# ToKe79/nuts333

Measured on NVIDIA B200. Metric: rendered messages/sec (colour+swear+ban), higher is better.
Workload: dtype u8

## Files before the change

nuts333_b200/csrc/nutsb_kernels.cuh:

```cuda
#pragma once
#include "nutsb_common.cuh"


struct OpsView {
    i64 n;
    const u8  *text;
    const u64 *toff;
    const u8  *kind;
    const i32 *target;
    const i32 *except_user;
    const u8  *flags;
    const i32 *gate;
    const u8  *verdict;
};

struct PopView {
    i32 n_users, n_rooms, n_rooms_tot;
    const i32 *user_room;
    const i32 *user_cls;
    const i32 *user_slot;
    const i32 *slot_user;
    const u8  *slot_cf;
    const u8  *slot_lv;
    const i32 *room_slot_off;
// ... 864 lines not shown
#endif
#ifndef NUTSB_FAN_GROUP
#define NUTSB_FAN_GROUP 1
#endif
#define NUTSB_FAN_SMEM (NUTSB_FAN_ON_CAP + 80 + NUTSB_FAN_OFF_CAP + 80 + 16 * NUTSB_FAN_RUN_CAP)

struct FanoutArgs {
    const ItemDesc *items; const uint4 *runs;
    const u8 *slab; u64 off_base;
    u8 *out;
};

__device__ __forceinline__ void nutsb_fanout_block(const FanoutArgs &A, u32 item, u8 *s_dyn)
{
    u8 *const s_on = s_dyn;
    u8 *const s_off = s_dyn + NUTSB_FAN_ON_CAP + 80;
    uint4 *const s_run = (uint4 *)(s_dyn + NUTSB_FAN_ON_CAP + 80 + NUTSB_FAN_OFF_CAP + 80);
    const int tid = threadIdx.x, warp = tid >> 5;
    const ItemDesc d = A.items[item];
    const bool staged = d.on_len <= NUTSB_FAN_ON_CAP && d.off_len <= NUTSB_FAN_OFF_CAP;
    const u32 a_on = (u32)(d.on_src & 15), a_off = (u32)(d.off_src & 15);
    if (staged) {
        const uint4 *g = (const uint4 *)(A.slab + (d.on_src - a_on));
        for (u32 v = (u32)tid, nv = (a_on + d.on_len + 15) >> 4; v < nv; v += NUTSB_FAN_THREADS) ((uint4 *)s_on)[v] = __ldg(g + v);
        g = (const uint4 *)(A.slab + (d.off_src - a_off));
        for (u32 v = (u32)tid, nv = (a_off + d.off_len + 15) >> 4; v < nv; v += NUTSB_FAN_THREADS) ((uint4 *)s_off)[v] = __ldg(g + v);
    }
    for (u32 r0 = 0; r0 < d.run_cnt; r0 += NUTSB_FAN_RUN_CAP) {
        const u32 nr = d.run_cnt - r0 < NUTSB_FAN_RUN_CAP ? d.run_cnt - r0 : NUTSB_FAN_RUN_CAP;
        if (r0) __syncthreads();
        for (u32 r = (u32)tid; r < nr; r += NUTSB_FAN_THREADS) s_run[r] = __ldg(A.runs + d.run_begin + r0 + r);
        __syncthreads();
        for (u32 r = (u32)warp / NUTSB_FAN_GROUP; r < nr; r += NUTSB_FAN_THREADS / 32 / NUTSB_FAN_GROUP) {
            const uint4 run = s_run[r];
            const u64 so = (u64)run.z | ((u64)(run.w >> 24) << 32);
            const u32 len = run.w & 0xffffffu;
            u8 *dst = A.out + (((u64)run.y << 32) | run.x);
            const u8 *src;
            if (!staged) src = A.slab + so;
            else if (so >= A.off_base) src = s_off + a_off + (u32)(so - d.off_src);
            else src = s_on + a_on + (u32)(so - d.on_src);
            nutsb_group_copy<32 * NUTSB_FAN_GROUP>(dst, src, len, tid % (32 * NUTSB_FAN_GROUP));
        }
    }
}

__global__ void __launch_bounds__(NUTSB_FAN_THREADS, NUTSB_FAN_MINBLOCKS)
k_fanout(FanoutArgs A)
{
    NUTSB_DYN_SMEM(s_dyn);
    nutsb_fanout_block(A, blockIdx.x, s_dyn);
}

struct DirectArgs {
    OpsView ops; PopView pop; ClassPrefix cpx;
    const u32 *room_b_off, *ev_off;
    const u32 *sv_ukey, *sv_op; const u64 *sv_pre;
    const u64 *stream_off;
    const u32 *ev_slot_sorted;
    const i32 *sv_delta;
    u8 *out; i64 n_ev;
    u64 *n_deliveries;
    u32 *status;
    const u8 *slab; u64 off_base;
    u32 has_level;
    const SlotInfo *slots;
    const u64 *dpre;
};

#define NUTSB_DIRECT_THREADS 256

struct DirectSink {
    u8 *out; u64 p; u32 O, osz;
    u32 cnt, done, qf;
    __device__ __forceinline__ void on(const u8 *w, u32 nbytes, int lane)
    {
        const u32 end = done + nbytes;
        while (qf < cnt) {
            const u32 Oq = __shfl_sync(NUTSB_FULL, O, (int)qf), zq = __shfl_sync(NUTSB_FULL, osz, (int)qf);
            const u64 pq = __shfl_sync(NUTSB_FULL, p, (int)qf);
            if (Oq >= end && zq) break;
            const u32 x0 = Oq > done ? Oq : done, x1 = Oq + zq < end ? Oq + zq : end;
            if (x1 > x0) {
                u8 *dst = out + pq + (x0 - Oq);
                const u8 *src = w + (x0 - done);
                const u32 len = x1 - x0;
                if (len < 192) { for (u32 i = (u32)lane; i < len; i += 32) dst[i] = src[i]; }
                else nutsb_warp_copy(dst, src, len, lane);
            }
            if (Oq + zq <= end) ++qf; else break;
        }
        done = end;
    }
    __device__ __forceinline__ void off(const u8 *, u32, int) {}
};

#define NUTSB_DIR_WARPS (NUTSB_DIRECT_THREADS / 32)
#define NUTSB_DIR_SMEM  (NUTSB_DIR_WARPS * (NUTSB_REN_ON_WIN + 64) + NUTSB_DIR_WARPS * 32 * (8 + 8 + 8) + ((NUTSB_CODETAB_BYTES + 15) & ~15))

template <bool COMPACT>
__device__ __forceinline__ void nutsb_direct_block(const DirectArgs &A, u32 blk, u32 nblk, u8 *smem)
{
    typedef u8 OnWin[NUTSB_REN_ON_WIN + 64];
    OnWin *const s_on = (OnWin *)smem;
    u64 (*const s_gw)[32] = (u64 (*)[32])(smem + NUTSB_DIR_WARPS * (NUTSB_REN_ON_WIN + 64));
    u64 (*const s_p)[32] = s_gw + NUTSB_DIR_WARPS;
    u32 (*const s_par)[32][2] = (u32 (*)[32][2])(s_p + NUTSB_DIR_WARPS);
    u8 *const s_tab = (u8 *)(s_par + NUTSB_DIR_WARPS);
    const int tid = threadIdx.x, lane = tid & 31, warp = tid >> 5;
    for (int i = tid; i < NUTSB_CODETAB_BYTES; i += NUTSB_DIRECT_THREADS) s_tab[i] = A.pop.codetab[i];
    __syncthreads();

    u64 c_cnt = 0, c_bytes = 0; u32 seam_bytes = 0;
    for (i64 ebase = ((i64)blk * (NUTSB_DIRECT_THREADS / 32) + warp) * 32; ebase < A.n_ev;
         ebase += (i64)nblk * NUTSB_DIRECT_THREADS) {
        const i64 e = ebase + lane;
        bool isw = false, seam = false, first_ev = false, last_ev = false;
        u64 p = 0, q = 0, gw = 0; u32 n = 0, al = 0, osz = 0, fl = 0;
        u64 a_start = 0, b_end = 0; const u8 *sa = nullptr, *sb = nullptr;
        if (e < A.n_ev) {
            const u32 uk = A.sv_ukey[e];
            const SlotInfo si = A.slots[A.ev_slot_sorted[e]];
            const u32 room = si.room; const i32 k = si.k;
            const u32 b0 = si.b0, cf = si.cf_lv & 0xffu;
            const u32 e0 = si.e0, e1 = si.e1;
            const u64 so_u = si.so_u, base = si.base;
            const u32 j = uk >> 2, ek = uk & 3u, skip = ek != NUTSB_EV_DIRECT;
            p = base + A.cpx.at(k, room, b0 + j) + A.sv_pre[e];
            q = base + A.cpx.at(k, room, b0 + j + skip) + A.sv_pre[e + 1];
            if (ek != NUTSB_EV_SKIP) {
                const u32 op = A.sv_op[e];
                const u64 t0 = A.ops.toff[op];
                const u8 *src = A.ops.text + t0;
                n = (u32)(A.ops.toff[op + 1] - t0);
                al = (u32)((size_t)src & 3);
                gw = (u64)(size_t)(src - al);
                nutsb_prefetch(src, n);
                fl = A.ops.flags[op] | ((cf & NUTSB_UF_COLOUR) ? NUTSB_FL_COLOUR : 0u);
                osz = (u32)(q - p);
                isw = true;
            }
            seam = !COMPACT && !A.has_level && !(cf & NUTSB_UF_FILTERED);
            if (COMPACT && isw) p = A.dpre[e];
            if (seam) {
                const bool colour = (cf & NUTSB_UF_COLOUR) != 0;
                const u64 *vp = colour ? A.cpx.vp_on : A.cpx.vp_off;
                const u8 *R = A.slab + (colour ? 0 : A.off_base);
                first_ev = (u32)e == e0; last_ev = (u32)e + 1 == e1;
                a_start = so_u; b_end = si.end;
                if (!first_ev && lane == 0) {
                    const u32 ukp = A.sv_ukey[e - 1];
                    a_start = base + A.cpx.at(k, room, b0 + (ukp >> 2) + ((ukp & 3u) != NUTSB_EV_DIRECT)) + A.sv_pre[e];
                }
                if (!last_ev && (lane == 31 || e + 1 >= A.n_ev))
                    b_end = base + A.cpx.at(k, room, b0 + (A.sv_ukey[e + 1] >> 2)) + A.sv_pre[e + 1];
                sa = R + vp[b0 + j];
                sb = R + vp[b0 + j + skip];
            }
        }
        if (!COMPACT) {
            const u64 q_prev = __shfl_up_sync(NUTSB_FULL, q, 1), p_next = __shfl_down_sync(NUTSB_FULL, p, 1);
            if (seam && !first_ev && lane > 0) a_start = q_prev;
            if (seam && !last_ev && lane < 31 && e + 1 < A.n_ev) b_end = p_next;
            u64 t0 = p & ~(u64)31; if (t0 < a_start) t0 = a_start;
            u64 h1 = (q + 31) & ~(u64)31; if (h1 > b_end) h1 = b_end;
            const u32 tlen = seam ? (u32)(p - t0) : 0u, hlen = seam && h1 > q ? (u32)(h1 - q) : 0u;
            seam_bytes += tlen + hlen;
            u8 *const stage = s_on[warp];
            const u32 lens = tlen | (hlen << 8);
            if (__any_sync(NUTSB_FULL, lens != 0)) {
#pragma unroll 8
                for (int i = 0; i < 32; ++i) {
                    const u32 l = __shfl_sync(NUTSB_FULL, lens, i);
                    const u8 *pa = (const u8 *)(size_t)__shfl_sync(NUTSB_FULL, (u64)(size_t)sa, i) - (l & 0xffu);
                    const u8 *pb = (const u8 *)(size_t)__shfl_sync(NUTSB_FULL, (u64)(size_t)sb, i);
                    u8 va = 0, vb = 0;
                    if ((u32)lane < (l & 0xffu)) va = pa[lane];
                    if ((u32)lane < (l >> 8)) vb = pb[lane];
                    stage[64 * i + lane] = va; stage[64 * i + 32 + lane] = vb;
                }
                __syncwarp();
#pragma unroll 4
                for (int i = 0; i < 32; ++i) {
                    const u32 l = __shfl_sync(NUTSB_FULL, lens, i);
                    const u64 da = __shfl_sync(NUTSB_FULL, t0, i), db = __shfl_sync(NUTSB_FULL, q, i);
                    if ((u32)lane < (l & 0xffu)) A.out[da + lane] = stage[64 * i + lane];
                    if ((u32)lane < (l >> 8)) A.out[db + lane] = stage[64 * i + 32 + lane];
                }
                __syncwarp();
            }
        }
        const u32 wmask = __ballot_sync(NUTSB_FULL, isw);
        const u32 cnt = (u32)__popc(wmask);
        if (!cnt) continue;
        if (isw) {
            const u32 r = (u32)__popc(wmask & ((1u << lane) - 1));
            s_gw[warp][r] = gw; s_p[warp][r] = p;
            s_par[warp][r][0] = NUTSB_FLAT_META(al, n, fl); s_par[warp][r][1] = osz;
        }
        __syncwarp();
        u32 nw = 0, meta = 0;
        osz = 0; gw = 0; p = 0;
        if ((u32)lane < cnt) {
            gw = s_gw[warp][lane]; p = s_p[warp][lane];
            meta = s_par[warp][lane][0]; osz = s_par[warp][lane][1];
            nw = ((meta & 3u) + ((meta >> 2) & 0xfffu) + 3) >> 2; if (!nw) nw = 1;
        }
        __syncwarp();
        u32 inc = osz;
        for (int d = 1; d < 32; d <<= 1) { const u32 t = __shfl_up_sync(NUTSB_FULL, inc, d); if (lane >= d) inc += t; }
        const u32 total = __shfl_sync(NUTSB_FULL, inc, 31);
        DirectSink sink{ A.out, p, inc - osz, osz, cnt, 0u, 0u };
        nutsb_flat_render<false>(cnt, meta, gw, nw, s_on[warp], (u8 *)nullptr, s_tab, lane, sink);
        if (lane == 0 && sink.done != total) atomicOr(A.status, NUTSB_ST_RENDER_MISMATCH);
        c_cnt += cnt; c_bytes += total;
    }
    for (int d = 16; d; d >>= 1) seam_bytes += __shfl_xor_sync(NUTSB_FULL, seam_bytes, d);
    if (lane == 0 && (c_cnt | seam_bytes)) { nutsb_add64(A.n_deliveries, c_cnt); nutsb_add64(A.n_deliveries + 1, c_bytes + seam_bytes); }
}

#ifndef NUTSB_DIR_MINBLOCKS
#define NUTSB_DIR_MINBLOCKS 5
#endif
__global__ void __launch_bounds__(NUTSB_DIRECT_THREADS, NUTSB_DIR_MINBLOCKS)
k_direct(DirectArgs A)
{
    NUTSB_DYN_SMEM(s_dyn);
    nutsb_direct_block<false>(A, blockIdx.x, gridDim.x, s_dyn);
}

__global__ void __launch_bounds__(NUTSB_DIRECT_THREADS, NUTSB_DIR_MINBLOCKS)
k_direct_compact(DirectArgs A)
{
    NUTSB_DYN_SMEM(s_dyn);
    nutsb_direct_block<true>(A, blockIdx.x, gridDim.x, s_dyn);
}

#define NUTSB_FD_SMEM (NUTSB_FAN_SMEM > NUTSB_DIR_SMEM ? NUTSB_FAN_SMEM : NUTSB_DIR_SMEM)
static_assert(NUTSB_FAN_THREADS == NUTSB_DIRECT_THREADS, "k_fanout_direct runs both bodies with one block size");
#ifndef NUTSB_FD_MINBLOCKS
#define NUTSB_FD_MINBLOCKS 5
#endif
__global__ void __launch_bounds__(NUTSB_FAN_THREADS, NUTSB_FD_MINBLOCKS)
k_fanout_direct(FanoutArgs F, DirectArgs D, u32 n_dir, u32 stride)
{
    NUTSB_DYN_SMEM(s_dyn);
    const u32 b = blockIdx.x;
    if (b % stride == 0 && b / stride < n_dir) { nutsb_direct_block<false>(D, b / stride, n_dir, s_dyn); return; }
    const u32 before = (b + stride - 1) / stride;
    nutsb_fanout_block(F, b - (before < n_dir ? before : n_dir), s_dyn);
}

__global__ void k_readback_end(const u64 *counters, const u32 *status, u64 *h_counters, u32 *h_status)
{
    if (threadIdx.x < 3) h_counters[threadIdx.x] = counters[threadIdx.x];
    if (threadIdx.x == 0) *h_status = *status;
}

#define NUTSB_DIGEST_P  0x100000001b3ull
#define NUTSB_DIGEST_H0 0xcbf29ce484222325ull

__global__ void __launch_bounds__(256)
k_digest(const u8 *bytes, const u64 *off, i32 n_users, const u64 *init, u64 *digest)
{
    __shared__ u64 s_m[256], s_a[256];
    for (i32 u = blockIdx.x; u < n_users; u += gridDim.x) {
        const u64 b = off[u], n = off[u + 1] - b;
        const u64 per = (n + 255) / 256;
        u64 lo = (u64)threadIdx.x * per, hi = lo + per;
        if (lo > n) lo = n;
        if (hi > n) hi = n;
        u64 m = 1, a = 0;
        for (u64 i = lo; i < hi; ++i) { m *= NUTSB_DIGEST_P; a = a * NUTSB_DIGEST_P + bytes[b + i]; }
        s_m[threadIdx.x] = m; s_a[threadIdx.x] = a;
        __syncthreads();
        if (threadIdx.x == 0) {
            u64 h = init ? init[u] : NUTSB_DIGEST_H0;
            for (int q = 0; q < 256; ++q) h = h * s_m[q] + s_a[q];
            digest[u] = h;
        }
        __syncthreads();
    }
}

__global__ void __launch_bounds__(64)
k_readback1(const u64 *eoff_end, const u32 *status, const u64 *slab_tot, u64 *h_entries, u32 *h_status, u64 *h_slab_tot)
{
    const u32 t = threadIdx.x;
    if (t == 0) { *h_entries = *eoff_end; *h_status = *status; }
    if (t < 2 * NUTSB_SLAB_TOT_WAYS) h_slab_tot[t] = slab_tot[t];
}

struct Sizes {
    u64 total_bytes;
    u64 cells;
    u64 slab_on, slab_off;
    u32 n_slab, n_events, items, tiles;
    u64 direct_bytes;
};

__global__ void __launch_bounds__(NUTSB_SCAN_THREADS)
// ... 216 lines not shown
```

nuts333_b200/csrc/nutsb_lib.cu:

```cuda
#include "nutsb_kernels.cuh"
#include "nutsb_match.cuh"
#include "nutsb_speech.cuh"

#define NUTSB_API extern "C" __attribute__((visibility("default")))

#include <algorithm>
#include <cstdio>
#include <cstdlib>
#include <cstring>
#include <deque>
#include <new>
#include <numeric>
#include <string>
#include <vector>

struct DBuf {
    void *p = nullptr; size_t cap = 0;
    template <class T> T *as() const { return (T *)p; }
};
struct HBuf {
    void *p = nullptr; size_t cap = 0;
    template <class T> T *as() const { return (T *)p; }
};

struct AcHost {
    std::vector<u32> trans; u8 clsmap[256]; u32 ncls = 1, nstates = 1, root_match = 0;
    std::vector<u16> tr16; u8 cls2[256]; u32 thresh = 0x10000u, maxpat = 0;
    std::vector<u16> t2; u16 clsA[256]; u8 clsB[256]; u32 t2_rs = 0;
};
struct AcDev { DBuf trans, clsmap, tr16, cls2, t2, clsA, clsB; AcView view{}; bool present = false; };
struct SetDev { DBuf slot_off, slot_len, pool; SetView view{}; bool present = false; };

struct ClassSet {
    std::vector<i32> user_cls, room_cls_off; std::vector<u8> cls_flags, cls_level;
    DBuf d_user_cls, d_room_cls_off, d_cls_flags, d_cls_level;
    i32 n_cls = 0, max_per_room = 0;
};

struct nutsb_ctx {
    int device = 0;
    cudaStream_t stream = nullptr; bool own_stream = true;
    cudaStream_t side = nullptr; bool overlap = true;
    int side_render = 8;
    int fd_dir_per_sm = 0;
    cudaEvent_t dep[4] = {nullptr, nullptr, nullptr, nullptr};
    int sm_count = 148;
    std::string err;
    bool profiling = false; nutsb_timing tm{};
    cudaEvent_t ev[12] = {};

    DBuf d_codetab;
    AcDev swear, site; SetDev userban;
    bool site_file = false, user_file = false;
    std::vector<u8> ban_bytes[2];

    bool have_users = false, all_simple = true, has_clones = false;
    i32 n_clone_flag = 0, n_remote_flag = 0;
    i32 U = 0, R = 0, Rt = 1;
    std::vector<i32> user_room, user_slot, slot_user, room_slot_off;
    std::vector<u8> uflags, ulevel;
    std::vector<i32> remote_link; std::vector<u8> remote_old;
    std::vector<i32> remotes;
    std::vector<i32> clone_owner; std::vector<u8> clone_hear;
    std::vector<std::vector<i32>> room_clones;
    std::vector<std::string> room_names;
    DBuf d_user_room, d_user_slot, d_slot_user, d_room_slot_off, d_slot_cf, d_slot_lv;
    ClassSet cls[2];

    DBuf d_status, d_len_on, d_len_off, d_nrep, d_eoff, d_sums, d_scan_ticket;
    void *scan_state_seen = nullptr; size_t scan_state_cap = 0; u32 scan_epoch = 0;
    DBuf d_ek[2], d_ev_[2];
    DBuf d_hist, d_hoffs;
    DBuf d_room_ent_off, d_e_info, d_e_delta, d_e_slot, d_e_scan, d_counts, d_room_b_off;
    DBuf d_bl_op, d_bl_room, d_evk[2], d_evv[2], d_ev_ukey, d_ev_delta, d_ev_op;
    DBuf d_sv_ukey, d_sv_delta, d_sv_op, d_sv_pre, d_ev_off;
    DBuf d_vp_on, d_vp_off, d_cp;
    DBuf d_room_tile_off, d_room_cell_off, d_room_item_off, d_sizes, d_counters;
    DBuf d_runs, d_items, d_slab, d_bl_meta, d_slots;
    DBuf d_off, d_out, d_digest, d_ulen;
    DBuf d_dpre, d_dir, d_iov, d_iov_first, d_iov_cnt;
    HBuf h_small, h_off, h_out, h_dir, h_iov, h_iov_first, h_iov_cnt;
    u64 last_total = 0; bool have_streams = false;
    struct LastBatch { bool valid = false; OpsView ops{}; ClassPrefix cpx{}; bool has_level = false; u64 off_base = 0; u32 *sv_slot = nullptr; } last;
    DBuf d_room_users, d_room_users_off, d_dg;

    DBuf s_text, s_toff, s_kind, s_target, s_except, s_flags, s_gate, s_verdict, s_v8;

    bool have_names = false; bool ban_swearing = false;
    std::vector<u8> names, sflags; std::vector<u64> name_off;
    std::vector<std::string> lits;
    DBuf d_names, d_name_off, d_sflags, d_lit, d_lit_off;
    DBuf d_sp_len, d_sp_off, d_sp_text, d_sp_kind, d_sp_target, d_sp_except, d_sp_flags, d_sp_gate, d_sp_verdict;
    DBuf s_verb, s_speaker, s_body, s_boff;

    std::vector<u8> q_text; std::vector<u64> q_off{0}; std::vector<u8> q_kind, q_flags;
    std::vector<i32> q_target, q_except, q_gate;
    std::vector<u8> q_sw_text; std::vector<u64> q_sw_off{0};
    std::vector<u8> q_sw_verdict;

    struct RevBuf { char buf[NUTSB_REVIEW_LINES][NUTSB_REVIEW_LEN + 2]; int line; };
    struct PendingRec { i32 room, gate; std::string text; };
    struct TellBuf { char buf[NUTSB_REVTELL_LINES][NUTSB_REVIEW_LEN + 2]; int line; };
    std::vector<TellBuf> revtell;
    std::vector<RevBuf> rev;
    std::vector<PendingRec> q_rec;
};

static int fail(nutsb_ctx *c, int code, const char *fmt, const char *a = "")
{
    if (c) { char b[512]; snprintf(b, sizeof b, fmt, a); c->err = b; }
    return code;
}
#define CK(call) do { cudaError_t e_ = (call); if (e_ != cudaSuccess) \
    return fail(c, e_ == cudaErrorMemoryAllocation ? NUTSB_E_NOMEM : NUTSB_E_CUDA, #call ": %s", cudaGetErrorString(e_)); } while (0)
#define CKL() CK(cudaGetLastError())
#define TRY(x) do { int r_ = (x); if (r_ != NUTSB_OK) return r_; } while (0)

static int ensure(nutsb_ctx *c, DBuf &b, size_t bytes)
{
    bytes = (bytes + 255) & ~(size_t)255;
    if (bytes + 256 <= b.cap) return NUTSB_OK;
    if (b.p) { CK(cudaStreamSynchronize(c->stream)); CK(cudaFree(b.p)); b.p = nullptr; b.cap = 0; }
    size_t want = bytes + bytes / 8 + 512;
    CK(cudaMalloc(&b.p, want));
    b.cap = want;
    return NUTSB_OK;
}
static int ensure_host(nutsb_ctx *c, HBuf &b, size_t bytes)
{
    if (bytes + 64 <= b.cap) return NUTSB_OK;
    if (b.p) { CK(cudaStreamSynchronize(c->stream)); CK(cudaFreeHost(b.p)); b.p = nullptr; b.cap = 0; }
// ... 201 lines not shown
    return NUTSB_OK;
}

static int ban_tokens(nutsb_ctx *c, const u8 *f, size_t n, std::vector<std::string> &out)
{
    auto ws = [](u8 b) { return b == ' ' || (b >= 9 && b <= 13); };
    size_t p = 0;
    while (true) {
        while (p < n && ws(f[p])) ++p;
        if (p >= n) break;
        const size_t b = p;
        while (p < n && !ws(f[p])) ++p;
        if (p >= n) break;
        if (p - b > NUTSB_MAX_BAN_TOKEN) return fail(c, NUTSB_E_RANGE, "ban token longer than 81 bytes%s");
        size_t m = 0; while (m < p - b && f[b + m]) ++m;
        out.emplace_back((const char *)f + b, m);
    }
    return NUTSB_OK;
}

NUTSB_API int nutsb_version(void) { return NUTSB_VERSION; }

NUTSB_API const char *nutsb_strerror(int code)
{
    switch (code) {
    case NUTSB_OK: return "ok";
    case NUTSB_E_INVAL: return "invalid argument";
    case NUTSB_E_NOMEM: return "out of memory";
    case NUTSB_E_CUDA: return "CUDA error";
    case NUTSB_E_UNSUPPORTED: return "unsupported recipient type (remote)";
    case NUTSB_E_RANGE: return "value out of range";
    case NUTSB_E_STATE: return "call order";
    }
    return "unknown";
}
NUTSB_API const char *nutsb_last_error(const nutsb_ctx *c) { return c ? c->err.c_str() : ""; }

NUTSB_API void nutsb_destroy(nutsb_ctx *c)
{
    if (!c) return;
    cudaSetDevice(c->device);
    if (c->stream) cudaStreamSynchronize(c->stream);
    DBuf *all[] = { &c->d_codetab, &c->swear.trans, &c->swear.clsmap, &c->swear.tr16, &c->swear.cls2, &c->site.trans, &c->site.clsmap, &c->site.tr16, &c->site.cls2,
        &c->userban.slot_off, &c->userban.slot_len, &c->userban.pool,
        &c->d_user_room, &c->d_user_slot, &c->d_slot_user, &c->d_room_slot_off, &c->d_slot_cf, &c->d_slot_lv,
        &c->cls[0].d_user_cls, &c->cls[0].d_room_cls_off, &c->cls[0].d_cls_flags, &c->cls[0].d_cls_level,
        &c->cls[1].d_user_cls, &c->cls[1].d_room_cls_off, &c->cls[1].d_cls_flags, &c->cls[1].d_cls_level,
        &c->d_status, &c->d_len_on, &c->d_len_off, &c->d_nrep, &c->d_eoff, &c->d_sums, &c->d_scan_ticket, &c->d_ek[0], &c->d_ek[1],
        &c->d_ev_[0], &c->d_ev_[1], &c->d_hist, &c->d_hoffs, &c->d_room_ent_off, &c->d_e_info, &c->d_e_delta,
        &c->d_e_slot, &c->d_e_scan, &c->d_counts, &c->d_room_b_off, &c->d_bl_op, &c->d_bl_room, &c->d_evk[0],
        &c->d_evk[1], &c->d_evv[0], &c->d_evv[1], &c->d_ev_ukey, &c->d_ev_delta, &c->d_ev_op, &c->d_sv_ukey,
        &c->d_sv_delta, &c->d_sv_op, &c->d_sv_pre, &c->d_ev_off, &c->d_vp_on, &c->d_vp_off, &c->d_cp,
        &c->d_room_tile_off, &c->d_room_cell_off, &c->d_room_item_off, &c->d_sizes, &c->d_counters,
        &c->d_runs, &c->d_slots, &c->d_items, &c->d_slab, &c->d_bl_meta, &c->d_off, &c->d_out, &c->d_digest, &c->d_ulen,
        &c->d_dpre, &c->d_dir, &c->d_iov, &c->d_iov_first, &c->d_iov_cnt, &c->d_room_users, &c->d_room_users_off, &c->d_dg,
        &c->s_text, &c->s_toff, &c->s_kind, &c->s_target, &c->s_except, &c->s_flags, &c->s_gate, &c->s_verdict, &c->s_v8,
        &c->d_names, &c->d_name_off, &c->d_sflags, &c->d_lit, &c->d_lit_off, &c->d_sp_len, &c->d_sp_off, &c->d_sp_text,
        &c->d_sp_kind, &c->d_sp_target, &c->d_sp_except, &c->d_sp_flags, &c->d_sp_gate, &c->d_sp_verdict,
        &c->s_verb, &c->s_speaker, &c->s_body, &c->s_boff };
    for (DBuf *b : all) release(*b);
    release(c->h_small); release(c->h_off); release(c->h_out);
    release(c->h_dir); release(c->h_iov); release(c->h_iov_first); release(c->h_iov_cnt);
    for (auto &e : c->ev) if (e) cudaEventDestroy(e);
    for (auto &e : c->dep) if (e) cudaEventDestroy(e);
    if (c->side) { cudaStreamSynchronize(c->side); cudaStreamDestroy(c->side); }
    if (c->own_stream && c->stream) cudaStreamDestroy(c->stream);
    delete c;
}

static int set_swear_impl(nutsb_ctx *c, const char *const *words)
{
    std::vector<std::string> pats;
    for (size_t i = 0; words && words[i] && words[i][0] != '*'; ++i) pats.emplace_back(words[i]);
    AcHost h; build_ac(pats, true, h);
    return upload_ac(c, h, c->swear);
}

NUTSB_API int nutsb_create(nutsb_ctx **out, int device)
{
    if (!out) return NUTSB_E_INVAL;
    *out = nullptr;
    int ndev = 0;
    if (cudaGetDeviceCount(&ndev) != cudaSuccess || ndev <= 0 || device < 0 || device >= ndev) return NUTSB_E_CUDA;
    nutsb_ctx *c = new (std::nothrow) nutsb_ctx;
    if (!c) return NUTSB_E_NOMEM;
    c->device = device;
    int rc = [&]() -> int {
        CK(cudaSetDevice(device));
        int prio_least = 0, prio_greatest = 0;
        CK(cudaDeviceGetStreamPriorityRange(&prio_least, &prio_greatest));
        CK(cudaStreamCreateWithPriority(&c->stream, cudaStreamNonBlocking, prio_greatest));
        CK(cudaDeviceGetAttribute(&c->sm_count, cudaDevAttrMultiProcessorCount, device));
        CK(cudaStreamCreateWithPriority(&c->side, cudaStreamNonBlocking, prio_least));
        if (const char *e = getenv("NUTSB_SIDE_RENDER")) c->side_render = std::max(1, atoi(e));
        if (const char *e = getenv("NUTSB_OVERLAP")) c->overlap = atoi(e) != 0;
        if (const char *e = getenv("NUTSB_FD_DIR_PER_SM")) c->fd_dir_per_sm = std::max(0, atoi(e));
        for (auto &e : c->ev) CK(cudaEventCreate(&e));
        for (auto &e : c->dep) CK(cudaEventCreateWithFlags(&e, cudaEventDisableTiming));
        CK(cudaFuncSetAttribute(k_fanout, cudaFuncAttributeMaxDynamicSharedMemorySize, NUTSB_FAN_SMEM));
        CK(cudaFuncSetAttribute(k_fanout_direct, cudaFuncAttributeMaxDynamicSharedMemorySize, NUTSB_FD_SMEM));
        CK(cudaFuncSetAttribute(k_direct, cudaFuncAttributeMaxDynamicSharedMemorySize, NUTSB_DIR_SMEM));
        CK(cudaFuncSetAttribute(k_ac_pair<true>, cudaFuncAttributeMaxDynamicSharedMemorySize, NUTSB_ACP_SMEM(0x4000)));
        CK(cudaFuncSetAttribute(k_ac_pair<false>, cudaFuncAttributeMaxDynamicSharedMemorySize, NUTSB_ACP_SMEM(2 * NUTSB_AC_SMEM_ENTRIES)));
        u8 tab[NUTSB_CODETAB_BYTES]; build_codetab(tab);
        TRY(upload(c, c->d_codetab, tab, sizeof tab));
        TRY(ensure(c, c->d_status, 64)); TRY(ensure(c, c->d_counts, 64)); TRY(ensure(c, c->d_sizes, sizeof(Sizes)));
        TRY(ensure(c, c->d_counters, 1024));
// ... 370 lines not shown
    if (!alias) {
        const i32 J = std::max(1, cs.max_per_room);
        TRY(ensure(c, c->d_cp, (size_t)J * (E + 1) * 8));
        for (i32 j = 0; j < J; ++j) {
            InClassLen in{ ops, c->d_bl_op.as<u32>(), c->d_bl_room.as<u32>(), len_on, len_off, pop.room_cls_off, pop.cls_flags, pop.cls_level, j };
            TRY(run_scan(c, in, OutU64{c->d_cp.as<u64>() + (size_t)j * (E + 1)}, (i64)E, counts));
        }
        cpx.cp = c->d_cp.as<u64>();
    }

    const bool par = c->overlap && c->side != nullptr;
    cudaStream_t sd = par ? c->side : st;
    u64 *counters = c->d_counters.as<u64>();
    if (off_base + slab_off >= (1ull << 40)) return fail(c, NUTSB_E_RANGE, "more than 2^40 bytes of rendered slab in one batch%s");
    TRY(ensure(c, c->d_slab, off_base + slab_off + 256));
    if (compact) TRY(ensure_host(c, c->h_out, (size_t)(off_base + slab_off) + 64));
    c->tm.slab_bytes = slab_on + slab_off;
    if (par) { CK(cudaEventRecord(c->dep[0], st)); CK(cudaStreamWaitEvent(sd, c->dep[0], 0)); }
    if (c->profiling) CK(cudaEventRecord(c->ev[1], sd));
    {
        RenderArgs ra{ ops, c->d_codetab.as<u8>(), c->d_bl_op.as<u32>(), c->d_vp_on.as<u64>(), c->d_vp_off.as<u64>(), counts,
                       c->d_slab.as<u8>(), off_base, counters, c->d_status.as<u32>() };
        u32 grid = cdiv(E, NUTSB_REN_OPS * (NUTSB_REN_THREADS / 32));
        if (par) grid = std::min(grid, (u32)(c->sm_count * c->side_render));
        NUTSB_LAUNCH(grid, NUTSB_REN_THREADS, sd, k_render, ra); CKL();
        c->tm.launches++;
    }
    if (c->profiling) CK(cudaEventRecord(c->ev[8], sd));
    if (compact && off_base + slab_off) CK(cudaMemcpyAsync(c->h_out.p, c->d_slab.p, (size_t)(off_base + slab_off), cudaMemcpyDeviceToHost, sd));
    if (par) CK(cudaEventRecord(c->dep[1], sd));

    u32 *sv_slot = nullptr, *perm = nullptr;
    TRY(radix_sort(c, c->d_evk, c->d_evv, (i64)E, counts + 1, bits_for((u64)std::max(U, 1)), &sv_slot, &perm));
    TRY(ensure(c, c->d_sv_ukey, E * 4 + 16)); TRY(ensure(c, c->d_sv_delta, E * 4 + 16)); TRY(ensure(c, c->d_sv_op, E * 4 + 16));
    TRY(ensure(c, c->d_sv_pre, (E + 2) * 8)); TRY(ensure(c, c->d_ev_off, ((size_t)U + 2) * 4));
    NUTSB_LAUNCH(cdiv(E + 1, 256), 256, st, k_ev_gather, perm, counts + 1, c->d_ev_ukey.as<u32>(), c->d_ev_delta.as<i32>(),
                 c->d_ev_op.as<u32>(), c->d_sv_ukey.as<u32>(), c->d_sv_delta.as<i32>(), c->d_sv_op.as<u32>(), sv_slot, (u32)U, c->d_ev_off.as<u32>()); CKL();
    TRY(run_scan(c, InI32{c->d_sv_delta.as<i32>()}, OutU64{c->d_sv_pre.as<u64>()}, (i64)E, counts + 1));
    c->tm.launches += 1;

    UserLenIn uli{ cpx, pop, c->d_room_b_off.as<u32>(), c->d_ev_off.as<u32>(), c->d_sv_pre.as<u64>() };
    TRY(run_scan(c, uli, OutU64{c->d_off.as<u64>()}, (i64)U, nullptr));
    TRY(ensure(c, c->d_slots, ((size_t)U + 1) * sizeof(SlotInfo)));
    if (U > 0) {
        SlotInfoArgs sa{ pop, cpx, c->d_room_b_off.as<u32>(), c->d_ev_off.as<u32>(), c->d_sv_pre.as<u64>(), c->d_off.as<u64>(), c->d_slots.as<SlotInfo>() };
        NUTSB_LAUNCH(cdiv((u64)U, 128), 128, st, k_slot_info, sa); CKL();
        c->tm.launches++;
    }
    if (compact) {
        TRY(ensure(c, c->d_dpre, (E + 2) * 8));
        TRY(run_scan(c, InDirectLen{ c->d_sv_ukey.as<u32>(), sv_slot, c->d_sv_delta.as<i32>(), c->d_slots.as<SlotInfo>(),
                                     c->d_vp_on.as<u64>(), c->d_vp_off.as<u64>() }, OutU64{c->d_dpre.as<u64>()}, (i64)E, counts + 1));
    }
    TRY(ensure(c, c->d_room_tile_off, ((size_t)Rt + 2) * 4)); TRY(ensure(c, c->d_room_cell_off, ((size_t)Rt + 2) * 8));
    TRY(ensure(c, c->d_room_item_off, ((size_t)Rt + 2) * 4));
    Sizes *hs = (Sizes *)(c->h_small.as<u8>() + 256);
    NUTSB_LAUNCH(1, NUTSB_SCAN_THREADS, st, k_geometry, pop, c->d_room_b_off.as<u32>(), c->d_off.as<u64>(), counts,
                 c->d_vp_on.as<u64>(), c->d_vp_off.as<u64>(),
                 c->d_room_tile_off.as<u32>(), c->d_room_cell_off.as<u64>(), c->d_room_item_off.as<u32>(), hs,
                 compact ? c->d_dpre.as<u64>() : (const u64 *)nullptr); CKL();
    c->tm.launches++;
    CK(cudaStreamSynchronize(st));
    const Sizes sz = *hs;
    if (sz.slab_on != slab_on || sz.slab_off != slab_off) return fail(c, NUTSB_E_CUDA, "internal: slab size mismatch%s");
    if (compact) {
        iv->compact = true;
        iv->slab_span = off_base + slab_off;
        iv->direct_bytes = sz.direct_bytes;
        iv->n_iov = 2ull * sz.n_events + (u64)U;
        TRY(ensure(c, c->d_dir, sz.direct_bytes + 64));
        TRY(ensure(c, c->d_iov, (size_t)iv->n_iov * sizeof(IovEnt)));
        TRY(ensure(c, c->d_iov_first, (size_t)U * 8)); TRY(ensure(c, c->d_iov_cnt, (size_t)U * 4));
        TRY(ensure_host(c, c->h_dir, (size_t)sz.direct_bytes + 64));
        TRY(ensure_host(c, c->h_iov, (size_t)iv->n_iov * sizeof(IovEnt)));
        TRY(ensure_host(c, c->h_iov_first, ((size_t)U + 1) * 8)); TRY(ensure_host(c, c->h_iov_cnt, ((size_t)U + 1) * 4));
        TRY(ensure_host(c, c->h_off, ((size_t)U + 1) * 8));
        if (c->profiling) { CK(cudaEventRecord(c->ev[9], st)); }
        if (sz.n_events > 0) {
            DirectArgs da{ ops, pop, cpx, c->d_room_b_off.as<u32>(), c->d_ev_off.as<u32>(), c->d_sv_ukey.as<u32>(), c->d_sv_op.as<u32>(),
                           c->d_sv_pre.as<u64>(), c->d_off.as<u64>(), sv_slot, c->d_sv_delta.as<i32>(), c->d_dir.as<u8>(), (i64)sz.n_events, counters,
                           c->d_status.as<u32>(), c->d_slab.as<u8>(), off_base, 0u, c->d_slots.as<SlotInfo>(), c->d_dpre.as<u64>() };
            NUTSB_LAUNCH_SMEM(cdiv(sz.n_events, NUTSB_DIRECT_THREADS), NUTSB_DIRECT_THREADS, NUTSB_DIR_SMEM, st, k_direct_compact, da); CKL();
            c->tm.launches++;
        }
        if (c->profiling) { CK(cudaEventRecord(c->ev[3], st)); CK(cudaEventRecord(c->ev[10], st)); }
        IovArgs ia{ pop, c->d_slots.as<SlotInfo>(), c->d_vp_on.as<u64>(), c->d_vp_off.as<u64>(), c->d_sv_ukey.as<u32>(), sv_slot,
                    c->d_dpre.as<u64>(), sz.n_events, (u64)(size_t)c->h_out.p, (u64)(size_t)c->h_dir.p, off_base,
                    c->d_iov.as<IovEnt>(), c->d_iov_first.as<u64>(), c->d_iov_cnt.as<u32>(), counters };
        NUTSB_LAUNCH(cdiv(std::max<u64>(sz.n_events, (u64)U), 256), 256, st, k_iov, ia); CKL();
        c->tm.launches++;
        if (c->profiling) { CK(cudaEventRecord(c->ev[2], st)); CK(cudaEventRecord(c->ev[11], st)); }
        if (sz.direct_bytes) CK(cudaMemcpyAsync(c->h_dir.p, c->d_dir.p, (size_t)sz.direct_bytes, cudaMemcpyDeviceToHost, st));
        CK(cudaMemcpyAsync(c->h_iov.p, c->d_iov.p, (size_t)iv->n_iov * sizeof(IovEnt), cudaMemcpyDeviceToHost, st));
        CK(cudaMemcpyAsync(c->h_iov_first.p, c->d_iov_first.p, (size_t)U * 8, cudaMemcpyDeviceToHost, st));
        CK(cudaMemcpyAsync(c->h_iov_cnt.p, c->d_iov_cnt.p, (size_t)U * 4, cudaMemcpyDeviceToHost, st));
        CK(cudaMemcpyAsync(c->h_off.p, c->d_off.p, ((size_t)U + 1) * 8, cudaMemcpyDeviceToHost, st));
        CK(cudaMemcpyAsync(h64 + 8, counters, 24, cudaMemcpyDeviceToHost, st));
        CK(cudaMemcpyAsync(h32 + 4, c->d_status.p, 4, cudaMemcpyDeviceToHost, st));
        if (par) CK(cudaStreamWaitEvent(st, c->dep[1], 0));
        if (c->profiling) CK(cudaEventRecord(c->ev[6], st));
        CK(cudaStreamSynchronize(st));
        TRY(status_to_error(c, h32[4]));
        c->last_total = sz.total_bytes; c->have_streams = false;
        if (c->profiling) {
            CK(cudaEventElapsedTime(&c->tm.plan_ms, c->ev[0], c->ev[9]));
            CK(cudaEventElapsedTime(&c->tm.render_ms, c->ev[1], c->ev[8]));
            CK(cudaEventElapsedTime(&c->tm.fanout_ms, c->ev[10], c->ev[2]));
            CK(cudaEventElapsedTime(&c->tm.direct_ms, c->ev[9], c->ev[3]));
            CK(cudaEventElapsedTime(&c->tm.total_ms, c->ev[0], c->ev[11]));
            CK(cudaEventElapsedTime(&c->tm.d2h_ms, c->ev[11], c->ev[6]));
        }
        c->tm.fanout_bytes_out = 0; c->tm.fanout_bytes_in = 0; c->tm.render_bytes_in = h64[10];
        out->n_users = U; out->total_bytes = sz.total_bytes; out->n_deliveries = h64[8];
        out->off = c->d_off.as<u64>(); out->bytes = nullptr; out->on_device = 1;
        return NUTSB_OK;
    }
    TRY(ensure(c, c->d_out, sz.total_bytes + 64));
    Geometry geo{ c->d_room_b_off.as<u32>(), c->d_room_tile_off.as<u32>(), c->d_room_cell_off.as<u64>(), c->d_room_item_off.as<u32>() };
    c->tm.fanout_launches = 0;

    const bool fan = sz.cells > 0 && sz.items > 0;
    const bool fused = par && fan && sz.n_events > 0;
    DirectArgs da{ ops, pop, cpx, c->d_room_b_off.as<u32>(), c->d_ev_off.as<u32>(), c->d_sv_ukey.as<u32>(), c->d_sv_op.as<u32>(),
                   c->d_sv_pre.as<u64>(), c->d_off.as<u64>(), sv_slot, c->d_sv_delta.as<i32>(), c->d_out.as<u8>(), (i64)sz.n_events, counters,
                   c->d_status.as<u32>(), c->d_slab.as<u8>(), off_base, has_level ? 1u : 0u, c->d_slots.as<SlotInfo>(), nullptr };
    u32 n_dir = cdiv(sz.n_events, NUTSB_DIRECT_THREADS);
    if (fused && c->fd_dir_per_sm > 0) n_dir = std::min(n_dir, (u32)(c->sm_count * c->fd_dir_per_sm));
    if (c->profiling) CK(cudaEventRecord(c->ev[9], sd));
    if (sz.n_events > 0 && !fused) {
        if (par) { CK(cudaEventRecord(c->dep[2], st)); CK(cudaStreamWaitEvent(sd, c->dep[2], 0)); }
        NUTSB_LAUNCH_SMEM(n_dir, NUTSB_DIRECT_THREADS, NUTSB_DIR_SMEM, sd, k_direct, da); CKL();
        c->tm.launches++;
    }
    if (c->profiling) CK(cudaEventRecord(c->ev[3], sd));
    if (par) CK(cudaEventRecord(c->dep[3], sd));

    if (fan) {
        TRY(ensure(c, c->d_items, (size_t)sz.items * sizeof(ItemDesc)));
        u32 *cursor = counts + 4;
        CK(cudaMemsetAsync(cursor, 0, 4, st));
        PlanArgs pa{ pop, geo, cpx, c->d_off.as<u64>(), c->d_ev_off.as<u32>(), c->d_sv_ukey.as<u32>(), c->d_sv_delta.as<i32>(),
                     c->d_sv_pre.as<u64>(), c->d_bl_meta.as<u32>(), (u64)sz.cells, off_base, has_level ? 1u : 0u,
                     c->d_slots.as<SlotInfo>(), cursor, nullptr, c->d_items.as<ItemDesc>(), counters, c->d_status.as<u32>() };
        u64 n_runs = sz.cells + sz.n_events;
        if (!alias) {
            NUTSB_LAUNCH(sz.items, NUTSB_UCHUNK, st, k_plan<false>, pa); CKL();
            CK(cudaMemcpyAsync(h32 + 6, cursor, 4, cudaMemcpyDeviceToHost, st));
            CK(cudaMemsetAsync(cursor, 0, 4, st));
            CK(cudaStreamSynchronize(st));
            n_runs = h32[6];
            c->tm.launches++;
        }
        if (n_runs >= 0xfffffff0ull) return fail(c, NUTSB_E_RANGE, "more than 2^32 copy runs in one batch%s");
        TRY(ensure(c, c->d_runs, (n_runs + 1) * sizeof(uint4)));
        pa.runs = c->d_runs.as<uint4>();
        NUTSB_LAUNCH(sz.items, NUTSB_UCHUNK, st, k_plan<true>, pa); CKL();
        c->tm.launches++;
    }

    if (par) CK(cudaStreamWaitEvent(st, c->dep[1], 0));
    if (c->profiling) CK(cudaEventRecord(c->ev[10], st));
    if (fan) {
        FanoutArgs fa{ c->d_items.as<ItemDesc>(), c->d_runs.as<uint4>(), c->d_slab.as<u8>(), off_base, c->d_out.as<u8>() };
        if (fused) {
            const u32 total = sz.items + n_dir;
            const u32 stride = std::max(1u, total / n_dir);
            NUTSB_LAUNCH_SMEM(total, NUTSB_FAN_THREADS, NUTSB_FD_SMEM, st, k_fanout_direct, fa, da, n_dir, stride); CKL();
        } else {
            NUTSB_LAUNCH_SMEM(sz.items, NUTSB_FAN_THREADS, NUTSB_FAN_SMEM, st, k_fanout, fa); CKL();
        }
        c->tm.launches++; c->tm.fanout_launches = 1;
    }
    if (c->profiling) CK(cudaEventRecord(c->ev[2], st));
    if (par) CK(cudaStreamWaitEvent(st, c->dep[3], 0));
    if (c->profiling) CK(cudaEventRecord(c->ev[11], st));

    NUTSB_LAUNCH(1, 32, st, k_readback_end, counters, c->d_status.as<u32>(), h64 + 8, h32 + 4); CKL();
    c->tm.launches++;
// ... 937 lines not shown
```

Baseline: 34.90 billion.

## Precompute per-event descriptors in a separate kernel ahead of direct render

Adds a k_ev_desc kernel that resolves each event's output position, text source, metadata and seam lengths and addresses into a packed 48-byte EvDesc array. The direct render kernel then reads one descriptor per lane instead of chasing slots, prefix tables and op offsets inline. When parallel streams are enabled and the path is not compact, the descriptor kernel runs on the side stream so it can overlap other planning work. In exchange it adds a kernel launch and an extra global write and read of the descriptor array, and it reuses dep[1] for the side-stream dependency.

```diff
diff --git a/nuts333_b200/csrc/nutsb_kernels.cuh b/nuts333_b200/csrc/nutsb_kernels.cuh
--- a/nuts333_b200/csrc/nutsb_kernels.cuh
+++ b/nuts333_b200/csrc/nutsb_kernels.cuh
@@ -940,20 +940,78 @@
     nutsb_fanout_block(A, blockIdx.x, s_dyn);
 }
 
+struct __align__(16) EvDesc {
+    u64 p;
+    u64 gw;
+    u64 tsrc, hsrc;
+    u32 osz;
+    u32 meta;
+    u32 lens;
+    u32 pad_;
+};
+#define NUTSB_ED_DIRECT 0x10000u
+
+struct EvDescArgs {
+    OpsView ops; ClassPrefix cpx;
+    const SlotInfo *slots;
+    const u32 *ev_slot_sorted;
+    const u32 *sv_ukey, *sv_op; const u64 *sv_pre;
+    const u32 *n_dev;
+    const u8 *slab; u64 off_base;
+    u32 has_level;
+    const u64 *dpre;
+    EvDesc *out;
+};
+
+__global__ void __launch_bounds__(256)
+k_ev_desc(EvDescArgs A)
+{
+    const i64 e = (i64)blockIdx.x * blockDim.x + threadIdx.x;
+    if (e >= (i64)*A.n_dev) return;
+    const u32 uk = A.sv_ukey[e];
+    const SlotInfo si = A.slots[A.ev_slot_sorted[e]];
+    const u32 cf = si.cf_lv & 0xffu;
+    const u32 j = uk >> 2, ek = uk & 3u, skip = ek != NUTSB_EV_DIRECT;
+    auto pos = [&](u32 g, i64 e2) -> u64 { return si.base + A.cpx.at(si.k, si.room, si.b0 + g) + A.sv_pre[e2]; };
+    const u64 p = pos(j, e), q = pos(j + skip, e + 1);
+    EvDesc d;
+    d.p = p; d.gw = 0; d.tsrc = 0; d.hsrc = 0; d.osz = (u32)(q - p); d.meta = 0; d.lens = 0; d.pad_ = 0;
+    if (ek != NUTSB_EV_SKIP) {
+        const u32 op = A.sv_op[e];
+        const u64 t0 = A.ops.toff[op];
+        const u8 *src = A.ops.text + t0;
+        const u32 al = (u32)((size_t)src & 3);
+        d.gw = (u64)(size_t)(src - al);
+        d.meta = NUTSB_FLAT_META(al, (u32)(A.ops.toff[op + 1] - t0), A.ops.flags[op] | ((cf & NUTSB_UF_COLOUR) ? NUTSB_FL_COLOUR : 0u));
+        d.lens = NUTSB_ED_DIRECT;
+        if (A.dpre) d.p = A.dpre[e];
+    }
+    if (!A.dpre && !A.has_level && !(cf & NUTSB_UF_FILTERED)) {
+        u64 a_start = si.so_u, b_end = si.end;
+        if ((u32)e != si.e0) {
+            const u32 ukp = A.sv_ukey[e - 1];
+            a_start = pos((ukp >> 2) + ((ukp & 3u) != NUTSB_EV_DIRECT), e);
+        }
+        if ((u32)e + 1 != si.e1) b_end = pos(A.sv_ukey[e + 1] >> 2, e + 1);
+        u64 t0 = p & ~(u64)31; if (t0 < a_start) t0 = a_start;
+        u64 h1 = (q + 31) & ~(u64)31; if (h1 > b_end) h1 = b_end;
+        const u32 tlen = (u32)(p - t0), hlen = h1 > q ? (u32)(h1 - q) : 0u;
+        const bool colour = (cf & NUTSB_UF_COLOUR) != 0;
+        const u64 *vp = colour ? A.cpx.vp_on : A.cpx.vp_off;
+        const u8 *R = A.slab + (colour ? 0 : A.off_base);
+        d.tsrc = (u64)(size_t)(R + vp[si.b0 + j] - tlen);
+        d.hsrc = (u64)(size_t)(R + vp[si.b0 + j + skip]);
+        d.lens |= tlen | (hlen << 8);
+    }
+    A.out[e] = d;
+}
+
 struct DirectArgs {
-    OpsView ops; PopView pop; ClassPrefix cpx;
-    const u32 *room_b_off, *ev_off;
-    const u32 *sv_ukey, *sv_op; const u64 *sv_pre;
-    const u64 *stream_off;
-    const u32 *ev_slot_sorted;
-    const i32 *sv_delta;
-    u8 *out; i64 n_ev;
+    const EvDesc *desc; i64 n_ev;
+    const u8 *codetab;
+    u8 *out;
     u64 *n_deliveries;
     u32 *status;
-    const u8 *slab; u64 off_base;
-    u32 has_level;
-    const SlotInfo *slots;
-    const u64 *dpre;
 };
 
 #define NUTSB_DIRECT_THREADS 256
@@ -986,7 +1044,6 @@
 #define NUTSB_DIR_WARPS (NUTSB_DIRECT_THREADS / 32)
 #define NUTSB_DIR_SMEM  (NUTSB_DIR_WARPS * (NUTSB_REN_ON_WIN + 64) + NUTSB_DIR_WARPS * 32 * (8 + 8 + 8) + ((NUTSB_CODETAB_BYTES + 15) & ~15))
 
-template <bool COMPACT>
 __device__ __forceinline__ void nutsb_direct_block(const DirectArgs &A, u32 blk, u32 nblk, u8 *smem)
 {
     typedef u8 OnWin[NUTSB_REN_ON_WIN + 64];
@@ -996,99 +1053,52 @@
     u32 (*const s_par)[32][2] = (u32 (*)[32][2])(s_p + NUTSB_DIR_WARPS);
     u8 *const s_tab = (u8 *)(s_par + NUTSB_DIR_WARPS);
     const int tid = threadIdx.x, lane = tid & 31, warp = tid >> 5;
-    for (int i = tid; i < NUTSB_CODETAB_BYTES; i += NUTSB_DIRECT_THREADS) s_tab[i] = A.pop.codetab[i];
+    for (int i = tid; i < NUTSB_CODETAB_BYTES; i += NUTSB_DIRECT_THREADS) s_tab[i] = A.codetab[i];
     __syncthreads();
 
     u64 c_cnt = 0, c_bytes = 0; u32 seam_bytes = 0;
     for (i64 ebase = ((i64)blk * (NUTSB_DIRECT_THREADS / 32) + warp) * 32; ebase < A.n_ev;
          ebase += (i64)nblk * NUTSB_DIRECT_THREADS) {
         const i64 e = ebase + lane;
-        bool isw = false, seam = false, first_ev = false, last_ev = false;
-        u64 p = 0, q = 0, gw = 0; u32 n = 0, al = 0, osz = 0, fl = 0;
-        u64 a_start = 0, b_end = 0; const u8 *sa = nullptr, *sb = nullptr;
-        if (e < A.n_ev) {
-            const u32 uk = A.sv_ukey[e];
-            const SlotInfo si = A.slots[A.ev_slot_sorted[e]];
-            const u32 room = si.room; const i32 k = si.k;
-            const u32 b0 = si.b0, cf = si.cf_lv & 0xffu;
-            const u32 e0 = si.e0, e1 = si.e1;
-            const u64 so_u = si.so_u, base = si.base;
-            const u32 j = uk >> 2, ek = uk & 3u, skip = ek != NUTSB_EV_DIRECT;
-            p = base + A.cpx.at(k, room, b0 + j) + A.sv_pre[e];
-            q = base + A.cpx.at(k, room, b0 + j + skip) + A.sv_pre[e + 1];
-            if (ek != NUTSB_EV_SKIP) {
-                const u32 op = A.sv_op[e];
-                const u64 t0 = A.ops.toff[op];
-                const u8 *src = A.ops.text + t0;
-                n = (u32)(A.ops.toff[op + 1] - t0);
-                al = (u32)((size_t)src & 3);
-                gw = (u64)(size_t)(src - al);
-                nutsb_prefetch(src, n);
-                fl = A.ops.flags[op] | ((cf & NUTSB_UF_COLOUR) ? NUTSB_FL_COLOUR : 0u);
-                osz = (u32)(q - p);
-                isw = true;
+        EvDesc d{};
+        if (e < A.n_ev) d = A.desc[e];
+        const bool isw = (d.lens & NUTSB_ED_DIRECT) != 0;
+        if (isw) nutsb_prefetch((const u8 *)(size_t)d.gw + (d.meta & 3u), (d.meta >> 2) & 0xfffu);
+        const u32 lens = d.lens & 0xffffu;
+        seam_bytes += (lens & 0xffu) + (lens >> 8);
+        if (__any_sync(NUTSB_FULL, lens != 0)) {
+            u8 *const stage = s_on[warp];
+            const u64 da = d.p - (lens & 0xffu), db = d.p + d.osz;
+#pragma unroll 8
+            for (int i = 0; i < 32; ++i) {
+                const u32 l = __shfl_sync(NUTSB_FULL, lens, i);
+                const u8 *pa = (const u8 *)(size_t)__shfl_sync(NUTSB_FULL, d.tsrc, i);
+                const u8 *pb = (const u8 *)(size_t)__shfl_sync(NUTSB_FULL, d.hsrc, i);
+                u8 va = 0, vb = 0;
+                if ((u32)lane < (l & 0xffu)) va = pa[lane];
+                if ((u32)lane < (l >> 8)) vb = pb[lane];
+                stage[64 * i + lane] = va; stage[64 * i + 32 + lane] = vb;
             }
-            seam = !COMPACT && !A.has_level && !(cf & NUTSB_UF_FILTERED);
-            if (COMPACT && isw) p = A.dpre[e];
-            if (seam) {
-                const bool colour = (cf & NUTSB_UF_COLOUR) != 0;
-                const u64 *vp = colour ? A.cpx.vp_on : A.cpx.vp_off;
-                const u8 *R = A.slab + (colour ? 0 : A.off_base);
-                first_ev = (u32)e == e0; last_ev = (u32)e + 1 == e1;
-                a_start = so_u; b_end = si.end;
-                if (!first_ev && lane == 0) {
-                    const u32 ukp = A.sv_ukey[e - 1];
-                    a_start = base + A.cpx.at(k, room, b0 + (ukp >> 2) + ((ukp & 3u) != NUTSB_EV_DIRECT)) + A.sv_pre[e];
-                }
-                if (!last_ev && (lane == 31 || e + 1 >= A.n_ev))
-                    b_end = base + A.cpx.at(k, room, b0 + (A.sv_ukey[e + 1] >> 2)) + A.sv_pre[e + 1];
-                sa = R + vp[b0 + j];
-                sb = R + vp[b0 + j + skip];
+            __syncwarp();
+#pragma unroll 4
+            for (int i = 0; i < 32; ++i) {
+                const u32 l = __shfl_sync(NUTSB_FULL, lens, i);
+                const u64 dai = __shfl_sync(NUTSB_FULL, da, i), dbi = __shfl_sync(NUTSB_FULL, db, i);
+                if ((u32)lane < (l & 0xffu)) A.out[dai + lane] = stage[64 * i + lane];
+                if ((u32)lane < (l >> 8)) A.out[dbi + lane] = stage[64 * i + 32 + lane];
             }
-        }
-        if (!COMPACT) {
-            const u64 q_prev = __shfl_up_sync(NUTSB_FULL, q, 1), p_next = __shfl_down_sync(NUTSB_FULL, p, 1);
-            if (seam && !first_ev && lane > 0) a_start = q_prev;
-            if (seam && !last_ev && lane < 31 && e + 1 < A.n_ev) b_end = p_next;
-            u64 t0 = p & ~(u64)31; if (t0 < a_start) t0 = a_start;
-            u64 h1 = (q + 31) & ~(u64)31; if (h1 > b_end) h1 = b_end;
-            const u32 tlen = seam ? (u32)(p - t0) : 0u, hlen = seam && h1 > q ? (u32)(h1 - q) : 0u;
-            seam_bytes += tlen + hlen;
-            u8 *const stage = s_on[warp];
-            const u32 lens = tlen | (hlen << 8);
-            if (__any_sync(NUTSB_FULL, lens != 0)) {
-#pragma unroll 8
-                for (int i = 0; i < 32; ++i) {
-                    const u32 l = __shfl_sync(NUTSB_FULL, lens, i);
-                    const u8 *pa = (const u8 *)(size_t)__shfl_sync(NUTSB_FULL, (u64)(size_t)sa, i) - (l & 0xffu);
-                    const u8 *pb = (const u8 *)(size_t)__shfl_sync(NUTSB_FULL, (u64)(size_t)sb, i);
-                    u8 va = 0, vb = 0;
-                    if ((u32)lane < (l & 0xffu)) va = pa[lane];
-                    if ((u32)lane < (l >> 8)) vb = pb[lane];
-                    stage[64 * i + lane] = va; stage[64 * i + 32 + lane] = vb;
-                }
-                __syncwarp();
-#pragma unroll 4
-                for (int i = 0; i < 32; ++i) {
-                    const u32 l = __shfl_sync(NUTSB_FULL, lens, i);
-                    const u64 da = __shfl_sync(NUTSB_FULL, t0, i), db = __shfl_sync(NUTSB_FULL, q, i);
-                    if ((u32)lane < (l & 0xffu)) A.out[da + lane] = stage[64 * i + lane];
-                    if ((u32)lane < (l >> 8)) A.out[db + lane] = stage[64 * i + 32 + lane];
-                }
-                __syncwarp();
-            }
+            __syncwarp();
         }
         const u32 wmask = __ballot_sync(NUTSB_FULL, isw);
         const u32 cnt = (u32)__popc(wmask);
         if (!cnt) continue;
         if (isw) {
             const u32 r = (u32)__popc(wmask & ((1u << lane) - 1));
-            s_gw[warp][r] = gw; s_p[warp][r] = p;
-            s_par[warp][r][0] = NUTSB_FLAT_META(al, n, fl); s_par[warp][r][1] = osz;
+            s_gw[warp][r] = d.gw; s_p[warp][r] = d.p;
+            s_par[warp][r][0] = d.meta; s_par[warp][r][1] = d.osz;
         }
         __syncwarp();
-        u32 nw = 0, meta = 0;
-        osz = 0; gw = 0; p = 0;
+        u32 nw = 0, meta = 0, osz = 0; u64 gw = 0, p = 0;
         if ((u32)lane < cnt) {
             gw = s_gw[warp][lane]; p = s_p[warp][lane];
             meta = s_par[warp][lane][0]; osz = s_par[warp][lane][1];
@@ -1096,14 +1106,14 @@
         }
         __syncwarp();
         u32 inc = osz;
-        for (int d = 1; d < 32; d <<= 1) { const u32 t = __shfl_up_sync(NUTSB_FULL, inc, d); if (lane >= d) inc += t; }
+        for (int dd = 1; dd < 32; dd <<= 1) { const u32 t = __shfl_up_sync(NUTSB_FULL, inc, dd); if (lane >= dd) inc += t; }
         const u32 total = __shfl_sync(NUTSB_FULL, inc, 31);
         DirectSink sink{ A.out, p, inc - osz, osz, cnt, 0u, 0u };
         nutsb_flat_render<false>(cnt, meta, gw, nw, s_on[warp], (u8 *)nullptr, s_tab, lane, sink);
         if (lane == 0 && sink.done != total) atomicOr(A.status, NUTSB_ST_RENDER_MISMATCH);
         c_cnt += cnt; c_bytes += total;
     }
-    for (int d = 16; d; d >>= 1) seam_bytes += __shfl_xor_sync(NUTSB_FULL, seam_bytes, d);
+    for (int dd = 16; dd; dd >>= 1) seam_bytes += __shfl_xor_sync(NUTSB_FULL, seam_bytes, dd);
     if (lane == 0 && (c_cnt | seam_bytes)) { nutsb_add64(A.n_deliveries, c_cnt); nutsb_add64(A.n_deliveries + 1, c_bytes + seam_bytes); }
 }
 
@@ -1114,14 +1124,7 @@
 k_direct(DirectArgs A)
 {
     NUTSB_DYN_SMEM(s_dyn);
-    nutsb_direct_block<false>(A, blockIdx.x, gridDim.x, s_dyn);
-}
-
-__global__ void __launch_bounds__(NUTSB_DIRECT_THREADS, NUTSB_DIR_MINBLOCKS)
-k_direct_compact(DirectArgs A)
-{
-    NUTSB_DYN_SMEM(s_dyn);
-    nutsb_direct_block<true>(A, blockIdx.x, gridDim.x, s_dyn);
+    nutsb_direct_block(A, blockIdx.x, gridDim.x, s_dyn);
 }
 
 #define NUTSB_FD_SMEM (NUTSB_FAN_SMEM > NUTSB_DIR_SMEM ? NUTSB_FAN_SMEM : NUTSB_DIR_SMEM)
@@ -1134,7 +1137,7 @@
 {
     NUTSB_DYN_SMEM(s_dyn);
     const u32 b = blockIdx.x;
-    if (b % stride == 0 && b / stride < n_dir) { nutsb_direct_block<false>(D, b / stride, n_dir, s_dyn); return; }
+    if (b % stride == 0 && b / stride < n_dir) { nutsb_direct_block(D, b / stride, n_dir, s_dyn); return; }
     const u32 before = (b + stride - 1) / stride;
     nutsb_fanout_block(F, b - (before < n_dir ? before : n_dir), s_dyn);
 }
diff --git a/nuts333_b200/csrc/nutsb_lib.cu b/nuts333_b200/csrc/nutsb_lib.cu
--- a/nuts333_b200/csrc/nutsb_lib.cu
+++ b/nuts333_b200/csrc/nutsb_lib.cu
@@ -43,7 +43,7 @@
     cudaStream_t side = nullptr; bool overlap = true;
     int side_render = 8;
     int fd_dir_per_sm = 0;
-    cudaEvent_t dep[4] = {nullptr, nullptr, nullptr, nullptr};
+    cudaEvent_t dep[5] = {nullptr, nullptr, nullptr, nullptr, nullptr};
     int sm_count = 148;
     std::string err;
     bool profiling = false; nutsb_timing tm{};
@@ -76,7 +76,7 @@
     DBuf d_sv_ukey, d_sv_delta, d_sv_op, d_sv_pre, d_ev_off;
     DBuf d_vp_on, d_vp_off, d_cp;
     DBuf d_room_tile_off, d_room_cell_off, d_room_item_off, d_sizes, d_counters;
-    DBuf d_runs, d_items, d_slab, d_bl_meta, d_slots;
+    DBuf d_runs, d_items, d_slab, d_bl_meta, d_slots, d_evdesc;
     DBuf d_off, d_out, d_digest, d_ulen;
     DBuf d_dpre, d_dir, d_iov, d_iov_first, d_iov_cnt;
     HBuf h_small, h_off, h_out, h_dir, h_iov, h_iov_first, h_iov_cnt;
@@ -384,7 +384,7 @@
         &c->d_evk[1], &c->d_evv[0], &c->d_evv[1], &c->d_ev_ukey, &c->d_ev_delta, &c->d_ev_op, &c->d_sv_ukey,
         &c->d_sv_delta, &c->d_sv_op, &c->d_sv_pre, &c->d_ev_off, &c->d_vp_on, &c->d_vp_off, &c->d_cp,
         &c->d_room_tile_off, &c->d_room_cell_off, &c->d_room_item_off, &c->d_sizes, &c->d_counters,
-        &c->d_runs, &c->d_slots, &c->d_items, &c->d_slab, &c->d_bl_meta, &c->d_off, &c->d_out, &c->d_digest, &c->d_ulen,
+        &c->d_runs, &c->d_slots, &c->d_evdesc, &c->d_items, &c->d_slab, &c->d_bl_meta, &c->d_off, &c->d_out, &c->d_digest, &c->d_ulen,
         &c->d_dpre, &c->d_dir, &c->d_iov, &c->d_iov_first, &c->d_iov_cnt, &c->d_room_users, &c->d_room_users_off, &c->d_dg,
         &c->s_text, &c->s_toff, &c->s_kind, &c->s_target, &c->s_except, &c->s_flags, &c->s_gate, &c->s_verdict, &c->s_v8,
         &c->d_names, &c->d_name_off, &c->d_sflags, &c->d_lit, &c->d_lit_off, &c->d_sp_len, &c->d_sp_off, &c->d_sp_text,
@@ -861,6 +861,17 @@
         TRY(run_scan(c, InDirectLen{ c->d_sv_ukey.as<u32>(), sv_slot, c->d_sv_delta.as<i32>(), c->d_slots.as<SlotInfo>(),
                                      c->d_vp_on.as<u64>(), c->d_vp_off.as<u64>() }, OutU64{c->d_dpre.as<u64>()}, (i64)E, counts + 1));
     }
+    TRY(ensure(c, c->d_evdesc, E * sizeof(EvDesc) + 16));
+    {
+        const bool side = par && !compact;
+        if (side) { CK(cudaEventRecord(c->dep[4], st)); CK(cudaStreamWaitEvent(sd, c->dep[4], 0)); }
+        EvDescArgs ed{ ops, cpx, c->d_slots.as<SlotInfo>(), sv_slot, c->d_sv_ukey.as<u32>(), c->d_sv_op.as<u32>(), c->d_sv_pre.as<u64>(),
+                       counts + 1, c->d_slab.as<u8>(), off_base, has_level ? 1u : 0u, compact ? c->d_dpre.as<u64>() : (const u64 *)nullptr,
+                       c->d_evdesc.as<EvDesc>() };
+        NUTSB_LAUNCH(cdiv(E, 256), 256, side ? sd : st, k_ev_desc, ed); CKL();
+        c->tm.launches++;
+        if (side) CK(cudaEventRecord(c->dep[1], sd));
+    }
     TRY(ensure(c, c->d_room_tile_off, ((size_t)Rt + 2) * 4)); TRY(ensure(c, c->d_room_cell_off, ((size_t)Rt + 2) * 8));
     TRY(ensure(c, c->d_room_item_off, ((size_t)Rt + 2) * 4));
     Sizes *hs = (Sizes *)(c->h_small.as<u8>() + 256);
@@ -886,10 +897,8 @@
         TRY(ensure_host(c, c->h_off, ((size_t)U + 1) * 8));
         if (c->profiling) { CK(cudaEventRecord(c->ev[9], st)); }
         if (sz.n_events > 0) {
-            DirectArgs da{ ops, pop, cpx, c->d_room_b_off.as<u32>(), c->d_ev_off.as<u32>(), c->d_sv_ukey.as<u32>(), c->d_sv_op.as<u32>(),
-                           c->d_sv_pre.as<u64>(), c->d_off.as<u64>(), sv_slot, c->d_sv_delta.as<i32>(), c->d_dir.as<u8>(), (i64)sz.n_events, counters,
-                           c->d_status.as<u32>(), c->d_slab.as<u8>(), off_base, 0u, c->d_slots.as<SlotInfo>(), c->d_dpre.as<u64>() };
-            NUTSB_LAUNCH_SMEM(cdiv(sz.n_events, NUTSB_DIRECT_THREADS), NUTSB_DIRECT_THREADS, NUTSB_DIR_SMEM, st, k_direct_compact, da); CKL();
+            DirectArgs da{ c->d_evdesc.as<EvDesc>(), (i64)sz.n_events, c->d_codetab.as<u8>(), c->d_dir.as<u8>(), counters, c->d_status.as<u32>() };
+            NUTSB_LAUNCH_SMEM(cdiv(sz.n_events, NUTSB_DIRECT_THREADS), NUTSB_DIRECT_THREADS, NUTSB_DIR_SMEM, st, k_direct, da); CKL();
             c->tm.launches++;
         }
         if (c->profiling) { CK(cudaEventRecord(c->ev[3], st)); CK(cudaEventRecord(c->ev[10], st)); }
@@ -930,9 +939,7 @@
 
     const bool fan = sz.cells > 0 && sz.items > 0;
     const bool fused = par && fan && sz.n_events > 0;
-    DirectArgs da{ ops, pop, cpx, c->d_room_b_off.as<u32>(), c->d_ev_off.as<u32>(), c->d_sv_ukey.as<u32>(), c->d_sv_op.as<u32>(),
-                   c->d_sv_pre.as<u64>(), c->d_off.as<u64>(), sv_slot, c->d_sv_delta.as<i32>(), c->d_out.as<u8>(), (i64)sz.n_events, counters,
-                   c->d_status.as<u32>(), c->d_slab.as<u8>(), off_base, has_level ? 1u : 0u, c->d_slots.as<SlotInfo>(), nullptr };
+    DirectArgs da{ c->d_evdesc.as<EvDesc>(), (i64)sz.n_events, c->d_codetab.as<u8>(), c->d_out.as<u8>(), counters, c->d_status.as<u32>() };
     u32 n_dir = cdiv(sz.n_events, NUTSB_DIRECT_THREADS);
     if (fused && c->fd_dir_per_sm > 0) n_dir = std::min(n_dir, (u32)(c->sm_count * c->fd_dir_per_sm));
     if (c->profiling) CK(cudaEventRecord(c->ev[9], sd));
```

After: 35.25 billion, median of 6. About the same (+1.0%).
